# maybeLx/MVSFormerPlusPlus

Hardware: AMD Instinct MI355X
Metric: ref-views/sec at 1152x1536 N=5 D=192 4-stage; achieved HBM GB/s vs peak (higher is better)
Workload: dtype fp16 operands/storage, fp32 accumulate (every stage; 1-2 fp16 MFMA terms)

## Files before the change

mvsformerplusplus_amd/csrc/vis_kernels.hip:

```cpp
#include "split_format.h"

namespace mvs {

constexpr int VS_TW = 60;
constexpr int VS_P = 64;
constexpr int VS_RING = 4;
constexpr int VS_SH_MAX = 64;
constexpr int VS_EP = VS_P + 2;
constexpr int VS_ENT_BYTES = (VS_SH_MAX + 6) * VS_EP * 4;
constexpr int VS_F16_PLANE_SHIFT = 0;
template <bool F16>
struct VsL {
    static constexpr int POSB = F16 ? 16 : 32;
    static constexpr int PLANE = ((VS_RING * VS_P + 2) * POSB + 255) / 256 * 256 + (F16 ? VS_F16_PLANE_SHIFT : 16);
    static constexpr int LAYER = 2 * PLANE;
    static constexpr int LDS = 2 * LAYER + VS_ENT_BYTES;
};
typedef _Float16 vs_f16x8 __attribute__((ext_vector_type(8)));
typedef _Float16 vs_f16x4 __attribute__((ext_vector_type(4)));

#ifndef MVS_OPAQUE_VEC
#define MVS_OPAQUE_VEC "v"
#endif

__device__ __forceinline__ vs_f16x4 vs_mask4(vs_f16x4 h, bool in) {
    typedef unsigned vs_u32x2 __attribute__((ext_vector_type(2)));
    vs_u32x2 u = __builtin_bit_cast(vs_u32x2, h);
    u[0] = in ? u[0] : 0u;
    u[1] = in ? u[1] : 0u;
    return __builtin_bit_cast(vs_f16x4, u);
}

__device__ __forceinline__ vs_f16x4 vs_cvt4(const float* v) {
    typedef float vs_f32x4 __attribute__((ext_vector_type(4)));
    return __builtin_convertvector((vs_f32x4){v[0], v[1], v[2], v[3]}, vs_f16x4);
}

template <int SLOT0, int POSB>
__device__ __forceinline__ int vs_step_off(int laneoff, int tapsel, int t) {
    const int tapA = 2 * t, tapB = 2 * t + 1 < 9 ? 2 * t + 1 : 8;
    const int offA = (((SLOT0 + tapA / 3) & (VS_RING - 1)) * VS_P + tapA % 3) * POSB;
    const int offB = (((SLOT0 + tapB / 3) & (VS_RING - 1)) * VS_P + tapB % 3) * POSB;
    return laneoff + (tapsel ? offB : offA);
}

struct VsOperand { bf16x8 h, l; };
template <bool F16>
__device__ __forceinline__ VsOperand vs_load(const char* p) {
    VsOperand o;
    o.h = *reinterpret_cast<const bf16x8*>(p);
    if constexpr (!F16) o.l = *reinterpret_cast<const bf16x8*>(p + 16);
    else o.l = o.h;
    return o;
}

template <bool F16>
__device__ __forceinline__ f32x4 vs_mfma_lo(const bf16x8& wl, const VsOperand& x, f32x4 a) {
    if constexpr (F16) return __builtin_amdgcn_mfma_f32_16x16x32_f16(__builtin_bit_cast(vs_f16x8, wl), __builtin_bit_cast(vs_f16x8, x.h), a, 0, 0, 0);
    else return __builtin_amdgcn_mfma_f32_16x16x32_bf16(wl, x.h, a, 0, 0, 0);
}
template <bool F16>
__device__ __forceinline__ f32x4 vs_mfma_hi(const bf16x8& wh, const VsOperand& x, f32x4 a) {
    if constexpr (F16) return __builtin_amdgcn_mfma_f32_16x16x32_f16(__builtin_bit_cast(vs_f16x8, wh), __builtin_bit_cast(vs_f16x8, x.h), a, 0, 0, 0);
    else return __builtin_amdgcn_mfma_f32_16x16x32_bf16(wh, x.h, a, 0, 0, 0);
}

template <int SLOT0, bool F16, bool ONE = false>
__device__ __forceinline__ f32x4 vs_layer_row(const char* lds_layer, int laneoff, int tapsel, const bf16x8* wh, const bf16x8* wl, f32x4 init) {
    constexpr int POSB = VsL<F16>::POSB;
    f32x4 a0 = {0.0f, 0.0f, 0.0f, 0.0f}, a1 = a0, a2 = init;
    VsOperand cur = vs_load<F16>(lds_layer + vs_step_off<SLOT0, POSB>(laneoff, tapsel, 0));
#pragma unroll
    for (int t = 0; t < 5; ++t) {
        VsOperand nxt = cur;
        if (t < 4) nxt = vs_load<F16>(lds_layer + vs_step_off<SLOT0, POSB>(laneoff, tapsel, t + 1));
        __builtin_amdgcn_sched_barrier(0);
        if constexpr (!ONE) a0 = vs_mfma_lo<F16>(wl[t], cur, a0);
        if constexpr (!F16) a1 = __builtin_amdgcn_mfma_f32_16x16x32_bf16(wh[t], cur.l, a1, 0, 0, 0);
        a2 = vs_mfma_hi<F16>(wh[t], cur, a2);
        cur = nxt;
    }
    return a0 + a1 + a2;
}

template <int SLOT2, int SLOT3, bool F16, bool ONE = false>
__device__ __forceinline__ void vs_two_layer_rows(const char* lds1, const char* lds2, int laneoff, int tapsel, const bf16x8* w2h,
                                                  const bf16x8* w2l, const bf16x8* w3h, const bf16x8* w3l, f32x4& out2, f32x4& out3) {
    constexpr int POSB = VsL<F16>::POSB;
    f32x4 a = out2, c = out3;
    VsOperand cb = vs_load<F16>(lds1 + vs_step_off<SLOT2, POSB>(laneoff, tapsel, 0));
    VsOperand cc = vs_load<F16>(lds2 + vs_step_off<SLOT3, POSB>(laneoff, tapsel, 0));
#pragma unroll
    for (int t = 0; t < 5; ++t) {
        VsOperand nb = cb, nc = cc;
        if (t < 4) {
            nb = vs_load<F16>(lds1 + vs_step_off<SLOT2, POSB>(laneoff, tapsel, t + 1));
            nc = vs_load<F16>(lds2 + vs_step_off<SLOT3, POSB>(laneoff, tapsel, t + 1));
        }
        __builtin_amdgcn_sched_barrier(0);
        if constexpr (!ONE) {
            a = vs_mfma_lo<F16>(w2l[t], cb, a);
            c = vs_mfma_lo<F16>(w3l[t], cc, c);
        }
        if constexpr (!F16) {
            a = __builtin_amdgcn_mfma_f32_16x16x32_bf16(w2h[t], cb.l, a, 0, 0, 0);
            c = __builtin_amdgcn_mfma_f32_16x16x32_bf16(w3h[t], cc.l, c, 0, 0, 0);
        }
        a = vs_mfma_hi<F16>(w2h[t], cb, a);
        c = vs_mfma_hi<F16>(w3h[t], cc, c);
        cb = nb;
        cc = nc;
    }
    out2 = a;
    out3 = c;
}

template <int V> struct VsInt { static constexpr int value = V; };

template <bool F16, bool ONE = false>
__global__ __launch_bounds__(256) void vis_cnn_kernel(const float* __restrict__ ent, const float* __restrict__ w1 ,
                                                      const float* __restrict__ b1, const void* __restrict__ wp2, const float* __restrict__ b2,
                                                      const void* __restrict__ wp3, const float* __restrict__ b3, const float* __restrict__ w4,
                                                      const float* __restrict__ b4, float* __restrict__ vis, int H, int W, int SH) {
    HIP_DYNAMIC_SHARED(float4, lds4)
    char* lds1 = reinterpret_cast<char*>(lds4);
    constexpr int VS_POSB = VsL<F16>::POSB, VS_PLANE = VsL<F16>::PLANE, VS_LAYER = VsL<F16>::LAYER;
    char* lds2 = lds1 + VS_LAYER;
    const int tid = (int)threadIdx.x, lane = tid & 63;
    const int wave = __builtin_amdgcn_readfirstlane(tid >> 6);
    const int li = lane & 15, g = lane >> 4;
    const int x0 = (int)blockIdx.x * VS_TW, r0 = (int)blockIdx.y * SH;
    const int r1 = r0 + SH < H ? r0 + SH : H;
    const float* e = ent + (size_t)blockIdx.z * H * W;
    float* vo = vis + (size_t)blockIdx.z * H * W;

    bf16x8 w2h[5], w2l[5], w3h[5], w3l[5];
    {
        const bf16x8* q2 = reinterpret_cast<const bf16x8*>(wp2) + lane;
        const bf16x8* q3 = reinterpret_cast<const bf16x8*>(wp3) + lane;
#pragma unroll
        for (int t = 0; t < 5; ++t) {
            w2h[t] = q2[(t * 2) * 64]; w2l[t] = q2[(t * 2 + 1) * 64];
            w3h[t] = q3[(t * 2) * 64]; w3l[t] = q3[(t * 2 + 1) * 64];
#ifndef MVS_NO_OPAQUE_VEC
            if constexpr (ONE) asm volatile("" : "+" MVS_OPAQUE_VEC(w2h[t]), "+" MVS_OPAQUE_VEC(w3h[t]));
            else asm volatile("" : "+" MVS_OPAQUE_VEC(w2h[t]), "+" MVS_OPAQUE_VEC(w2l[t]), "+" MVS_OPAQUE_VEC(w3h[t]), "+" MVS_OPAQUE_VEC(w3l[t]));
#endif
        }
    }
    constexpr bool L1MFMA = F16 && ONE;
    vs_f16x8 w1a = {0, 0, 0, 0, 0, 0, 0, 0};
    f32x4 b1q = {0.0f, 0.0f, 0.0f, 0.0f};
    if constexpr (L1MFMA) {
        const int kh = g < 3 ? g : 0;
#pragma unroll
        for (int kw = 0; kw < 3; ++kw) {
            const _Float16 wv = g < 3 ? (_Float16)w1[(kh * 3 + kw) * 16 + li] : (_Float16)0.0f;
            w1a[kw] = wv;
            w1a[3 + kw] = wv;
        }
#pragma unroll
        for (int r = 0; r < 4; ++r) b1q[r] = b1[4 * g + r];
    }
    float w1s[9][4], b1s[4];
#pragma unroll
    for (int t = 0; t < 9; ++t)
#pragma unroll
        for (int r = 0; r < 4; ++r) w1s[t][r] = w1[t * 16 + 4 * wave + r];
#pragma unroll
    for (int r = 0; r < 4; ++r) b1s[r] = b1[4 * wave + r];
    float b2v[4], b3v[4], w4v[4];
#pragma unroll
    for (int r = 0; r < 4; ++r) {
        b2v[r] = b2[4 * g + r];
        b3v[r] = g < 2 ? b3[4 * g + r] : 0.0f;
        w4v[r] = g < 2 ? w4[4 * g + r] : 0.0f;
    }
    const float bias4 = b4[0];

    const int xa = x0 - 2 + lane;
    const int i0 = r0 - 2, i1 = r1 + 4;
    float* ent_s = reinterpret_cast<float*>(lds1 + 2 * VS_LAYER);
    {
        const int nrow = r1 - r0 + 6;
        for (int idx = tid; idx < nrow * VS_EP; idx += 256) {
            const int rr = idx / VS_EP, cc = idx - rr * VS_EP;
            const int yy = r0 - 3 + rr, xx = x0 - 3 + cc;
            ent_s[idx] = (yy >= 0 && yy < H && xx >= 0 && xx < W) ? e[(size_t)yy * W + xx] : 0.0f;
        }
    }
    __syncthreads();
    const int colmaskA = xa >= 0 && xa < W;
    const int wrA = (wave >> 1) * VS_PLANE + lane * VS_POSB + (wave & 1) * 8;
    const int laneoff = (g & 1) * VS_PLANE + (16 * wave + li) * VS_POSB;
    const int wrB = (g >> 1) * VS_PLANE + (16 * wave + li) * VS_POSB + (g & 1) * 8;
    const int tapsel = g >> 1;
    const int c2 = 16 * wave + li;
    const int xb = x0 - 1 + c2, xc = x0 + c2;

    auto iteration = [&](auto phase, auto steady, int i) __attribute__((always_inline)) {
        constexpr int PH = decltype(phase)::value;
        constexpr bool STEADY = decltype(steady)::value != 0;
        if constexpr (L1MFMA) {
            if (STEADY || i <= r1 + 1) {
                const float* ep = ent_s + (i - 1 + (g < 3 ? g : 2) - (r0 - 3)) * VS_EP + c2;
                const float e0 = ep[0], e1 = ep[1], e2 = ep[2];
                typedef float vs_f32x2 __attribute__((ext_vector_type(2)));
                typedef _Float16 vs_f16x2 __attribute__((ext_vector_type(2)));
                typedef unsigned vs_u32x4 __attribute__((ext_vector_type(4)));
                const unsigned p0 = __builtin_bit_cast(unsigned, __builtin_convertvector((vs_f32x2){e0, e1}, vs_f16x2));
                const float l0 = MVS_FMA_MIX_LO(p0, -1.0f, e0), l1 = MVS_FMA_MIX_HI(p0, -1.0f, e1);
                const unsigned p1 = __builtin_bit_cast(unsigned, __builtin_convertvector((vs_f32x2){e2, l0}, vs_f16x2));
                const float l2 = MVS_FMA_MIX_LO(p1, -1.0f, e2);
                const unsigned p2 = __builtin_bit_cast(unsigned, __builtin_convertvector((vs_f32x2){l1, l2}, vs_f16x2));
                const vs_f16x8 bop = __builtin_bit_cast(vs_f16x8, (vs_u32x4){p0, p1, p2, 0u});
                const f32x4 r1v = __builtin_amdgcn_mfma_f32_16x16x32_f16(w1a, bop, b1q, 0, 0, 0);
                const int xa1 = x0 - 2 + c2;
                const bool in = xa1 >= 0 && xa1 < W && i >= 0 && i < H;
                float a[4];
#pragma unroll
                for (int r = 0; r < 4; ++r) a[r] = fmaxf(r1v[r], 0.0f);
                *reinterpret_cast<vs_f16x4*>(lds1 + wrB + PH * (VS_P * VS_POSB)) = vs_mask4(vs_cvt4(a), in);
            }
        } else if (STEADY || i <= r1 + 1) {
            float er[3][3];
            const float* ep = ent_s + (i - 1 - (r0 - 3)) * VS_EP + lane;
#pragma unroll
            for (int kh = 0; kh < 3; ++kh)
#pragma unroll
                for (int kw = 0; kw < 3; ++kw) er[kh][kw] = ep[kh * VS_EP + kw];
            typedef float f32x2 __attribute__((ext_vector_type(2)));
            f32x2 a01 = {b1s[0], b1s[1]}, a23 = {b1s[2], b1s[3]};
#pragma unroll
            for (int kh = 0; kh < 3; ++kh)
#pragma unroll
                for (int kw = 0; kw < 3; ++kw) {
                    const f32x2 ev = {er[kh][kw], er[kh][kw]};
                    a01 = __builtin_elementwise_fma(ev, (f32x2){w1s[kh * 3 + kw][0], w1s[kh * 3 + kw][1]}, a01);
                    a23 = __builtin_elementwise_fma(ev, (f32x2){w1s[kh * 3 + kw][2], w1s[kh * 3 + kw][3]}, a23);
                }
            float a[4] = {a01[0], a01[1], a23[0], a23[1]};
            const bool in = colmaskA && i >= 0 && i < H;
#pragma unroll
            for (int r = 0; r < 4; ++r) a[r] = F16 ? fmaxf(a[r], 0.0f) : (in ? fmaxf(a[r], 0.0f) : 0.0f);
            char* p = lds1 + wrA + PH * (VS_P * VS_POSB);
            if constexpr (F16) {
                *reinterpret_cast<vs_f16x4*>(p) = vs_mask4(vs_cvt4(a), in);
            } else {
                bf16x4 hi, lo;
                split4(a, hi, lo);
                *reinterpret_cast<bf16x4*>(p) = hi;
                *reinterpret_cast<bf16x4*>(p + 16) = lo;
            }
        }
        const int yb = i - 2, yc = i - 4;
        const bool doB = STEADY || (yb >= r0 - 1 && yb <= r1), doC = STEADY || yc >= r0;
        constexpr int S2 = (PH + 1) & 3, S3 = (PH + 3) & 3;
        f32x4 acc2 = {b2v[0], b2v[1], b2v[2], b2v[3]}, acc3 = {b3v[0], b3v[1], b3v[2], b3v[3]};
        if (STEADY || (doB && doC)) vs_two_layer_rows<S2, S3, F16, ONE>(lds1, lds2, laneoff, tapsel, w2h, w2l, w3h, w3l, acc2, acc3);
        else if (doB) acc2 = vs_layer_row<S2, F16, ONE>(lds1, laneoff, tapsel, w2h, w2l, acc2);
        else if (doC) acc3 = vs_layer_row<S3, F16, ONE>(lds2, laneoff, tapsel, w3h, w3l, acc3);
        if (doB) {
            const bool in = xb >= 0 && xb < W && yb >= 0 && yb < H;
            float v[4];
#pragma unroll
            for (int r = 0; r < 4; ++r) v[r] = F16 ? fmaxf(acc2[r], 0.0f) : (in ? fmaxf(acc2[r], 0.0f) : 0.0f);
            char* p = lds2 + wrB + ((PH + 2) & 3) * (VS_P * VS_POSB);
            if constexpr (F16) {
                *reinterpret_cast<vs_f16x4*>(p) = vs_mask4(vs_cvt4(v), in);
            } else {
                bf16x4 hi, lo;
                split4(v, hi, lo);
                *reinterpret_cast<bf16x4*>(p) = hi;
                *reinterpret_cast<bf16x4*>(p + 16) = lo;
            }
        }
        if (doC) {
            float part = 0.0f;
#pragma unroll
            for (int r = 0; r < 4; ++r) part += fmaxf(acc3[r], 0.0f) * w4v[r];
            part += __shfl_xor(part, 16);
            if (g == 0 && c2 < VS_TW && xc < W && yc < r1) {
                const float z = part + bias4;
                vo[(size_t)yc * W + xc] = __builtin_amdgcn_rcpf(1.0f + __builtin_amdgcn_exp2f(-z * 1.4426950408889634f));
            }
        }
        __syncthreads();
    };
    auto general = [&](int i) __attribute__((always_inline)) {
        switch (i & 3) {
            case 0: iteration(VsInt<0>(), VsInt<0>(), i); break;
            case 1: iteration(VsInt<1>(), VsInt<0>(), i); break;
            case 2: iteration(VsInt<2>(), VsInt<0>(), i); break;
            default: iteration(VsInt<3>(), VsInt<0>(), i); break;
        }
    };
    int i = i0;
    for (; i < i1 && (i < r0 + 4 || (i & 3) != 0); ++i) general(i);
    for (; i + 3 <= r1 + 1; i += 4) {
        iteration(VsInt<0>(), VsInt<1>(), i);
        iteration(VsInt<1>(), VsInt<1>(), i + 1);
        iteration(VsInt<2>(), VsInt<1>(), i + 2);
        iteration(VsInt<3>(), VsInt<1>(), i + 3);
    }
    for (; i < i1; ++i) general(i);
}


template <bool F16, bool ONE = false>
static int vis_weight_stream_t(const float* entropy, const float* w1, const float* b1, const void* w2, const float* b2, const void* w3,
                               const float* b3, const float* w4, const float* b4, float* vis, int N, int H, int W, hipStream_t st) {
    constexpr int VS_LDS = VsL<F16>::LDS;
    const int strips = (int)ceil_div(W, VS_TW);
    const long long per_seg = (long long)strips * N, resident = (160 * 1024 / VS_LDS < 4 ? 160 * 1024 / VS_LDS : 4) * 256;
    int segs = (int)ceil_div(H, VS_SH_MAX), SH = (int)ceil_div(H, segs);
    long long best = -1;
    for (int sg = (int)ceil_div(H, VS_SH_MAX); sg <= (H + 7) / 8; ++sg) {
        const int sh = (int)ceil_div(H, sg);
        const long long rounds = (per_seg * ceil_div(H, sh) + resident - 1) / resident;
        const long long cost = rounds * (sh + 6);
        if (best < 0 || cost < best) { best = cost; segs = (int)ceil_div(H, sh); SH = sh; }
    }
    if (VS_LDS > 48 * 1024)
        hipFuncSetAttribute(reinterpret_cast<const void*>(&vis_cnn_kernel<F16, ONE>), hipFuncAttributeMaxDynamicSharedMemorySize, VS_LDS);
    hipLaunchKernelGGL((vis_cnn_kernel<F16, ONE>), dim3(strips, segs, N), dim3(256), VS_LDS, st, entropy, w1, b1, w2, b2, w3, b3, w4, b4, vis, H, W, SH);
    return check_launch("vis_cnn_kernel");
}

int vis_weight_stream_bf16x3(const float* entropy, const float* w1, const float* b1, const void* w2, const float* b2, const void* w3,
                             const float* b3, const float* w4, const float* b4, float* vis, int N, int H, int W, hipStream_t st, int f16) {
    if (f16 == 2) return vis_weight_stream_t<true, true>(entropy, w1, b1, w2, b2, w3, b3, w4, b4, vis, N, H, W, st);
    return f16 ? vis_weight_stream_t<true>(entropy, w1, b1, w2, b2, w3, b3, w4, b4, vis, N, H, W, st)
               : vis_weight_stream_t<false>(entropy, w1, b1, w2, b2, w3, b3, w4, b4, vis, N, H, W, st);
}

}
```

Baseline: 688.6.

## Reuse each input row across three kernel rows via carried partial accumulators

For the fp16 single-term path, the layer-2 and layer-3 3x3 convolutions are restructured. Each LDS input row is loaded once and multiplied by all three kernel-row weight slices, and two partial accumulators per layer carry results across iterations instead of re-reading three input rows per output row. The prologue and epilogue iterations use a runtime phase instead of a four-way switch, which shrinks the code. The cost is extra accumulator registers and reliance on correct pipeline ordering in the boundary iterations, where the partial sums are now computed unconditionally.

```diff
diff --git a/mvsformerplusplus_amd/csrc/vis_kernels.hip b/mvsformerplusplus_amd/csrc/vis_kernels.hip
--- a/mvsformerplusplus_amd/csrc/vis_kernels.hip
+++ b/mvsformerplusplus_amd/csrc/vis_kernels.hip
@@ -115,6 +115,46 @@
     out3 = c;
 }
 
+struct VsReuseW { u32x4 a[3]; u32x2 b[3]; };
+
+__device__ __forceinline__ void vs_reuse_weights(const void* wp, int g, int li, VsReuseW& k) {
+    auto entry = [&](int o) { return ((o >> 2) * 2) * 64 + (o & 3) * 16 + li; };
+#pragma unroll
+    for (int kh = 0; kh < 3; ++kh) {
+        k.a[kh] = reinterpret_cast<const u32x4*>(wp)[entry(2 * (3 * kh + (g >> 1)) + (g & 1))];
+        k.b[kh] = reinterpret_cast<const u32x2*>(wp)[2 * entry(2 * (3 * kh + 2) + (g >> 1)) + (g & 1)];
+    }
+}
+
+__device__ __forceinline__ f32x4 vs_reuse_mfma(const u32x4& w, const vs_f16x8& x, f32x4 a) {
+    return __builtin_amdgcn_mfma_f32_16x16x32_f16(__builtin_bit_cast(vs_f16x8, w), x, a, 0, 0, 0);
+}
+__device__ __forceinline__ f32x4 vs_reuse_mfma(const u32x2& w, const vs_f16x4& x, f32x4 a) {
+    return __builtin_amdgcn_mfma_f32_16x16x16f16(__builtin_bit_cast(vs_f16x4, w), x, a, 0, 0, 0);
+}
+
+__device__ __forceinline__ void vs_reuse_rows(const char* lds1, const char* lds2, int slot2, int slot3, int off0, int off1, const VsReuseW& k2, const VsReuseW& k3,
+                                              f32x4& p2, f32x4& q2, f32x4& out2, f32x4& p3, f32x4& q3, f32x4& out3) {
+    constexpr int ROWB = VS_P * VsL<true>::POSB;
+    const vs_f16x8 x2a = *reinterpret_cast<const vs_f16x8*>(lds1 + off0 + slot2 * ROWB);
+    const vs_f16x8 x3a = *reinterpret_cast<const vs_f16x8*>(lds2 + off0 + slot3 * ROWB);
+    const vs_f16x4 x2b = *reinterpret_cast<const vs_f16x4*>(lds1 + off1 + slot2 * ROWB);
+    const vs_f16x4 x3b = *reinterpret_cast<const vs_f16x4*>(lds2 + off1 + slot3 * ROWB);
+    __builtin_amdgcn_sched_barrier(0);
+    f32x4 d2 = vs_reuse_mfma(k2.a[2], x2a, p2);
+    f32x4 d3 = vs_reuse_mfma(k3.a[2], x3a, p3);
+    f32x4 m2 = vs_reuse_mfma(k2.a[1], x2a, q2);
+    f32x4 m3 = vs_reuse_mfma(k3.a[1], x3a, q3);
+    f32x4 n2 = vs_reuse_mfma(k2.a[0], x2a, out2);
+    f32x4 n3 = vs_reuse_mfma(k3.a[0], x3a, out3);
+    out2 = vs_reuse_mfma(k2.b[2], x2b, d2);
+    out3 = vs_reuse_mfma(k3.b[2], x3b, d3);
+    p2 = vs_reuse_mfma(k2.b[1], x2b, m2);
+    p3 = vs_reuse_mfma(k3.b[1], x3b, m3);
+    q2 = vs_reuse_mfma(k2.b[0], x2b, n2);
+    q3 = vs_reuse_mfma(k3.b[0], x3b, n3);
+}
+
 template <int V> struct VsInt { static constexpr int value = V; };
 
 template <bool F16, bool ONE = false>
@@ -134,8 +174,18 @@
     const float* e = ent + (size_t)blockIdx.z * H * W;
     float* vo = vis + (size_t)blockIdx.z * H * W;
 
+    constexpr bool REUSE = F16 && ONE;
     bf16x8 w2h[5], w2l[5], w3h[5], w3l[5];
-    {
+    VsReuseW k2, k3;
+    if constexpr (REUSE) {
+        vs_reuse_weights(wp2, g, li, k2);
+        vs_reuse_weights(wp3, g, li, k3);
+#ifndef MVS_NO_OPAQUE_VEC
+#pragma unroll
+        for (int kh = 0; kh < 3; ++kh)
+            asm volatile("" : "+" MVS_OPAQUE_VEC(k2.a[kh]), "+" MVS_OPAQUE_VEC(k2.b[kh]), "+" MVS_OPAQUE_VEC(k3.a[kh]), "+" MVS_OPAQUE_VEC(k3.b[kh]));
+#endif
+    } else {
         const bf16x8* q2 = reinterpret_cast<const bf16x8*>(wp2) + lane;
         const bf16x8* q3 = reinterpret_cast<const bf16x8*>(wp3) + lane;
 #pragma unroll
@@ -195,11 +245,14 @@
     const int laneoff = (g & 1) * VS_PLANE + (16 * wave + li) * VS_POSB;
     const int wrB = (g >> 1) * VS_PLANE + (16 * wave + li) * VS_POSB + (g & 1) * 8;
     const int tapsel = g >> 1;
+    const int laneoff0 = laneoff + tapsel * VS_POSB, laneoff1 = wrB + 2 * VS_POSB;
+    f32x4 accP2 = {0.0f, 0.0f, 0.0f, 0.0f}, accQ2 = accP2, accP3 = accP2, accQ3 = accP2;
     const int c2 = 16 * wave + li;
     const int xb = x0 - 1 + c2, xc = x0 + c2;
 
     auto iteration = [&](auto phase, auto steady, int i) __attribute__((always_inline)) {
         constexpr int PH = decltype(phase)::value;
+        const int ph = PH >= 0 ? PH : (i & 3);
         constexpr bool STEADY = decltype(steady)::value != 0;
         if constexpr (L1MFMA) {
             if (STEADY || i <= r1 + 1) {
@@ -220,7 +273,7 @@
                 float a[4];
 #pragma unroll
                 for (int r = 0; r < 4; ++r) a[r] = fmaxf(r1v[r], 0.0f);
-                *reinterpret_cast<vs_f16x4*>(lds1 + wrB + PH * (VS_P * VS_POSB)) = vs_mask4(vs_cvt4(a), in);
+                *reinterpret_cast<vs_f16x4*>(lds1 + wrB + ph * (VS_P * VS_POSB)) = vs_mask4(vs_cvt4(a), in);
             }
         } else if (STEADY || i <= r1 + 1) {
             float er[3][3];
@@ -257,7 +310,9 @@
         const bool doB = STEADY || (yb >= r0 - 1 && yb <= r1), doC = STEADY || yc >= r0;
         constexpr int S2 = (PH + 1) & 3, S3 = (PH + 3) & 3;
         f32x4 acc2 = {b2v[0], b2v[1], b2v[2], b2v[3]}, acc3 = {b3v[0], b3v[1], b3v[2], b3v[3]};
-        if (STEADY || (doB && doC)) vs_two_layer_rows<S2, S3, F16, ONE>(lds1, lds2, laneoff, tapsel, w2h, w2l, w3h, w3l, acc2, acc3);
+        if constexpr (REUSE) {
+            vs_reuse_rows(lds1, lds2, (ph + 3) & 3, (ph + 1) & 3, laneoff0, laneoff1, k2, k3, accP2, accQ2, acc2, accP3, accQ3, acc3);
+        } else if (STEADY || (doB && doC)) vs_two_layer_rows<S2, S3, F16, ONE>(lds1, lds2, laneoff, tapsel, w2h, w2l, w3h, w3l, acc2, acc3);
         else if (doB) acc2 = vs_layer_row<S2, F16, ONE>(lds1, laneoff, tapsel, w2h, w2l, acc2);
         else if (doC) acc3 = vs_layer_row<S3, F16, ONE>(lds2, laneoff, tapsel, w3h, w3l, acc3);
         if (doB) {
@@ -265,7 +320,7 @@
             float v[4];
 #pragma unroll
             for (int r = 0; r < 4; ++r) v[r] = F16 ? fmaxf(acc2[r], 0.0f) : (in ? fmaxf(acc2[r], 0.0f) : 0.0f);
-            char* p = lds2 + wrB + ((PH + 2) & 3) * (VS_P * VS_POSB);
+            char* p = lds2 + wrB + ((ph + 2) & 3) * (VS_P * VS_POSB);
             if constexpr (F16) {
                 *reinterpret_cast<vs_f16x4*>(p) = vs_mask4(vs_cvt4(v), in);
             } else {
@@ -288,7 +343,8 @@
         __syncthreads();
     };
     auto general = [&](int i) __attribute__((always_inline)) {
-        switch (i & 3) {
+        if constexpr (REUSE) iteration(VsInt<-1>(), VsInt<0>(), i);
+        else switch (i & 3) {
             case 0: iteration(VsInt<0>(), VsInt<0>(), i); break;
             case 1: iteration(VsInt<1>(), VsInt<0>(), i); break;
             case 2: iteration(VsInt<2>(), VsInt<0>(), i); break;
```

Result: no change. 694.4 (median of 6 runs) (+0.9%).
